# commanderson/morna

Measured on AMD Instinct MI355X. Metric: samples indexed/sec (index build + 1000 queries, k=20) at 50k x 3000, higher is better.
Workload: dtype f32; 1 GPU; synthetic intropolis 50000 samples x 3000 features, 200 trees, 1000 by-item queries, k=20, search_k=100 (BASELINE.json configs[2]); samples_total=50000, samples_per_gpu=50000, features=3000, n_trees=200, queries=1000, k=20, search_k=100, nnz_per_gpu=100542830, junction_lines=70000

## Files before the change

### morna_amd/csrc/knn.hip

```cpp
#include <algorithm>
#include <cfloat>
#include <cstdint>
#include <cmath>
#include <cstring>
#include <type_traits>

#include "common.hpp"
#include "devutil.hpp"
#include "mm16.hpp"

namespace morna {

#define Q_THREADS 256
#define Q_WAVES (Q_THREADS / WAVE)
#define Q_MAX_DPAD 32768
#define Q_LDS_MAX (152 * 1024)

struct QueryParams {
    const float *X;
    const float *norm2;
    int64_t n_items;
    int32_t dpad, n_trees, K;
    const int32_t *node_rec;
    const int32_t *node_tree;
// ... 571 lines not shown
            }
            best = block_min_u64(best, s_red, tid);
            if (tid == 0) emit(r, best);
            prev = best;
        }
    }
    for (int r = kout + tid; r < P.k; r += Q_THREADS) {
        P.ids_out[qi * P.k + r] = -1;
        P.dist_out[qi * P.k + r] = INFINITY;
    }
    if (tid == 0) P.count_out[qi] = kout;
}

template <int BR, int BK, int NS>
__global__ __launch_bounds__(MM16_THREADS) void query_scores_kernel(const _Float16 *__restrict__ X16, int64_t n_items, int32_t dpad,
                                                                    const _Float16 *__restrict__ Q16,
                                                                    const int32_t *__restrict__ qrow, int32_t nq,
                                                                    float *__restrict__ scores, int64_t r_begin )
{
    extern __shared__ __attribute__((aligned(16))) unsigned char smem[];
    __shared__ int32_t s_qrow[MM16_TILE];
    constexpr int NB = BR / 128;
    const int tid = threadIdx.x, lane = tid & (WAVE - 1), w = tid / WAVE;
    const int wm = w >> 1, wn = w & 1;
    const int n_ct = (nq + MM16_TILE - 1) / MM16_TILE;
    const int64_t row_tile = (int64_t)((blockIdx.x >> 3) / n_ct) * 8 + (blockIdx.x & 7);
    const int64_t r0 = r_begin + row_tile * BR;
    const int c0 = (int)((blockIdx.x >> 3) % n_ct) * MM16_TILE;
    if (r0 >= n_items) return;
    if (tid < MM16_TILE) {
        const int q = c0 + tid < nq ? c0 + tid : nq - 1;
        s_qrow[tid] = qrow ? qrow[q] : q;
    }
    __syncthreads();
    mm16_f32x16 acc[NB][2];
    mm16_tile<BR, BK, NS>(X16, Q16, dpad, smem, [&](int rt) { return r0 + rt < n_items ? r0 + rt : n_items - 1; },
                          [&](int rt) { return (int64_t)s_qrow[rt]; }, acc);
    const int lr = lane & 31, lh = lane >> 5;
#pragma unroll
    for (int tb = 0; tb < NB; tb++) {
        const int64_t r = r0 + wm * 32 * NB + tb * 32 + lr;
        if (r < n_items) {
#pragma unroll
            for (int tn = 0; tn < 2; tn++)
#pragma unroll
                for (int e = 0; e < 16; e++) {
                    const int q = c0 + wn * 64 + tn * 32 + (e & 3) + 8 * (e >> 2) + 4 * lh;
                    if (q < nq) scores[(int64_t)q * n_items + r] = acc[tb][tn][e];
                }
        }
    }
}

template <int BK, int NS>
__global__ __launch_bounds__(1024) void query_scores_big_kernel(const _Float16 *__restrict__ X16, int64_t n_items, int32_t dpad,
                                                                const _Float16 *__restrict__ Q16, const int32_t *__restrict__ qrow,
                                                                int32_t nq, float *__restrict__ scores, int32_t n_row_tiles)
{
    extern __shared__ __attribute__((aligned(16))) unsigned char smem[];
    __shared__ int32_t s_qrow[256];
    const int tid = threadIdx.x, lane = tid & (WAVE - 1), w = tid / WAVE;
    const int wm = w >> 2, wn = w & 3;
    const int n_ct = (nq + 255) / 256;
    const int64_t row_tile = (int64_t)((blockIdx.x >> 3) / n_ct) * 8 + (blockIdx.x & 7);
    if (row_tile >= n_row_tiles) return;
    const int64_t r0 = row_tile * 256;
    const int c0 = (int)((blockIdx.x >> 3) % n_ct) * 256;
    if (tid < 256) {
        const int q = c0 + tid < nq ? c0 + tid : nq - 1;
        s_qrow[tid] = qrow ? qrow[q] : q;
    }
    __syncthreads();
    mm16_f32x16 acc[2][2];
    mm16_tile_256x256<BK, NS>(X16, Q16, dpad, smem, [&](int rt) { return r0 + rt; }, [&](int rt) { return (int64_t)s_qrow[rt]; }, acc);
    const int lr = lane & 31, lh = lane >> 5;
#pragma unroll
    for (int tb = 0; tb < 2; tb++) {
        const int64_t r = r0 + wm * 64 + tb * 32 + lr;
#pragma unroll
        for (int tn = 0; tn < 2; tn++)
#pragma unroll
            for (int e = 0; e < 16; e++) {
                const int q = c0 + wn * 64 + tn * 32 + (e & 3) + 8 * (e >> 2) + 4 * lh;
                if (q < nq) scores[(int64_t)q * n_items + r] = acc[tb][tn][e];
            }
    }
}

template <int MODE>
__global__ __launch_bounds__(Q_THREADS) void query_refine_kernel(QueryParams P)
{
    extern __shared__ __attribute__((aligned(16))) unsigned char smem[];
    float4 *qv = (float4 *)smem;
    __shared__ uint64_t s_red[Q_WAVES];
    __shared__ uint64_t s_top[Q_WAVES * KTH_MAX_K];
    __shared__ int s_nsurv;

    const int tid = threadIdx.x, lane = tid & (WAVE - 1), w = tid / WAVE;
    const int64_t qi = blockIdx.x;
    const int nvec = P.dpad / 4;
    const float4 *src = P.items ? (const float4 *)(P.X + (int64_t)P.items[qi] * P.dpad)
                                : (const float4 *)(P.Q + qi * P.dpad);
    for (int i = tid; i < nvec; i += Q_THREADS) qv[i] = src[i];
    if (tid == 0) s_nsurv = 0;
    __syncthreads();

    int32_t *cand = P.cand + qi * P.cap;
    uint64_t *keys = P.keys + qi * P.cap;
    const int ncand = P.ncand[qi] < P.cap ? P.ncand[qi] : P.cap;
    const float pp = P.qpp[qi];
    int nsel = ncand;

    if (MODE != 0 && ncand > P.k) {
        float *low = P.low + qi * P.cap;
        const float nan = __int_as_float(0x7fc00000);
        if (MODE == 1) {
            typedef _Float16 f16x8 __attribute__((ext_vector_type(8)));
            const int nv8 = P.dpad / 8;
            for (int c = w; c < ncand; c += Q_WAVES) {
                const int32_t id = cand[c];
                const f16x8 *y = (const f16x8 *)(P.X16 + (int64_t)id * P.dpad);
                float s0 = 0.f, s1 = 0.f, s2 = 0.f, s3 = 0.f;
                auto mac8 = [&](const f16x8 hv, int i) {
                    const float4 qa = qv[2 * i], qb = qv[2 * i + 1];
                    s0 = fmaf((float)hv[0], qa.x, s0);
                    s1 = fmaf((float)hv[1], qa.y, s1);
                    s2 = fmaf((float)hv[2], qa.z, s2);
                    s3 = fmaf((float)hv[3], qa.w, s3);
                    s0 = fmaf((float)hv[4], qb.x, s0);
                    s1 = fmaf((float)hv[5], qb.y, s1);
                    s2 = fmaf((float)hv[6], qb.z, s2);
                    s3 = fmaf((float)hv[7], qb.w, s3);
                };
                int i = lane;
                for (; i + 5 * WAVE < nv8; i += 6 * WAVE) {
                    const f16x8 h0 = y[i], h1 = y[i + WAVE], h2 = y[i + 2 * WAVE], h3 = y[i + 3 * WAVE];
// ... 292 lines not shown
            uint8_t *dp = (uint8_t *)h->host_small.dev();
            if (!dp) {
                set_error("query: the answer staging is not visible to the device");
                return MORNA_E_HIP;
            }
            P.ids_out = (int32_t *)dp;
            P.dist_out = (float *)(dp + s_ids);
            P.count_out = (int32_t *)(dp + 2 * s_ids);
        }
        if (spread) {
            ScopedTimer tm(h, MORNA_T_QUERY, 0);
            hipLaunchKernelGGL(query_roots_kernel, dim3((unsigned)((h->n_trees + Q_WAVES - 1) / Q_WAVES), (unsigned)nb), dim3(Q_THREADS), 0,
                               h->stream, P);
            MORNA_TRY(launch_descend(h->stream));
#ifdef MORNA_DESCEND_PROBE
            {
                float probe[40];
                HIP_TRY(hipStreamSynchronize(h->stream));
                HIP_TRY(hipMemcpy(probe, P.low + 2 * nb + 16, sizeof(probe), hipMemcpyDeviceToHost));
                fprintf(stderr, "[descend probe] cycles:");
                for (int i = 1; i < (int)probe[0] && i < 40; i++) fprintf(stderr, " %.0f", probe[i]);
                fprintf(stderr, "\n");
            }
#endif
            hipLaunchKernelGGL(query_cand_dots_kernel, dim3((unsigned)((cap + Q_WAVES * QS_CPW - 1) / (Q_WAVES * QS_CPW)), (unsigned)nb),
                               dim3(Q_THREADS), 0, h->stream, P);
            hipLaunchKernelGGL(query_topk_kernel, dim3((unsigned)nb), dim3(Q_THREADS), 0, h->stream, P);
        } else {
            ScopedTimer tm(h, MORNA_T_QUERY, 0);
            if (dense) {
                const _Float16 *q16 = P.X16;
                const int32_t *qrow = P.items;
                if (q_host) {
                    split_mm_convert_rows(h, Qd, nb, Q16, q_n16, q_e16, q_scale, h->stream);
                    q16 = Q16; qrow = nullptr;
                    P.qn16 = q_n16; P.qe16 = q_e16; P.qscale = q_scale;
                } else {
                    P.qn16 = P.xn16; P.qe16 = P.xe16; P.qscale = P.xscale;
                }
                HIP_TRY(hipEventRecord(h->ev_fork, h->stream));
                HIP_TRY(hipStreamWaitEvent(h->stream2, h->ev_fork, 0));
                ScopedTimer tf(h, MORNA_T_QUERY_FILTER, 2 * (int64_t)nb * N * h->dpad);
                static const bool big_on = env_on("MORNA_QUERY_BIG");
                int64_t big_tiles = 0;
                if (big_on && nb >= 512) {
                    const int64_t n_ct_big = (nb + 255) / 256;
                    int64_t a = h->n_cus, b = n_ct_big;
                    while (b) { const int64_t t = a % b; a = b; b = t; }
                    const int64_t per_round = h->n_cus / a;
                    big_tiles = (N / 256) / per_round * per_round;
                }
                if (big_tiles > 0) {
                    const unsigned n_ct_big = (unsigned)((nb + 255) / 256);
                    HIP_TRY(hipFuncSetAttribute((const void *)query_scores_big_kernel<64, 2>, hipFuncAttributeMaxDynamicSharedMemorySize, 128 * 256 * 4));
                    hipLaunchKernelGGL((query_scores_big_kernel<64, 2>), dim3(8u * (unsigned)((big_tiles + 7) / 8) * n_ct_big), dim3(1024), 128 * 256 * 4,
                                       h->stream, P.X16, N, h->dpad, q16, qrow, (int32_t)nb, scores, (int32_t)big_tiles);
                    P.big_rows = big_tiles * 256;
                    P.eacc_big = (4.f * (float)h->dpad + 2.f) * 5.9604645e-8f + 4.1e-6f;
                }
                if (P.big_rows < N) {
                    const unsigned n_ct = (unsigned)((nb + MM16_TILE - 1) / MM16_TILE), n_rt = (unsigned)((N - P.big_rows + 127) / 128);
                    HIP_TRY(hipFuncSetAttribute((const void *)query_scores_kernel<128, 64, 2>, hipFuncAttributeMaxDynamicSharedMemorySize, MM16_LDS));
                    hipLaunchKernelGGL((query_scores_kernel<128, 64, 2>), dim3(8u * ((n_rt + 7) / 8) * n_ct), dim3(MM16_THREADS), MM16_LDS,
                                       big_tiles > 0 ? h->stream2 : h->stream, P.X16, N, h->dpad, q16, qrow, (int32_t)nb, scores, P.big_rows);
                }
                P.scores = scores;
            }
            hipStream_t ts = dense ? h->stream2 : h->stream;
            const int nvq = h->dpad / 256;
            const bool nv_ok = h->dpad % 256 == 0 && (nvq == 1 || nvq == 2 || nvq == 3 || nvq == 4 || nvq == 6 || nvq == 8 || nvq == 12);
            const bool split_traverse = nv_ok && N > h->K && (size_t)QR_Q * h->dpad * 4 <= 128 * 1024 &&
                                        env_on("MORNA_QUERY_SPLIT_TRAVERSE");
            if (split_traverse) {
                const dim3 grid((unsigned)((nb + QR_Q - 1) / QR_Q), (unsigned)((h->n_trees + QR_TREES - 1) / QR_TREES));
                const size_t ql = (size_t)QR_Q * h->dpad * 4;
#define ROOTSB(NVV)                                                                                                      \
    do {                                                                                                                 \
        if (ql > 48 * 1024)                                                                                              \
            HIP_TRY(hipFuncSetAttribute((const void *)query_roots_batch_kernel<NVV>,                                      \
                                        hipFuncAttributeMaxDynamicSharedMemorySize, (int)ql));                           \
        hipLaunchKernelGGL((query_roots_batch_kernel<NVV>), grid, dim3(QR_THREADS), ql, ts, P, (int32_t)nb);             \
    } while (0)
                switch (nvq) {
                case 1: ROOTSB(1); break;
                case 2: ROOTSB(2); break;
                case 3: ROOTSB(3); break;
                case 4: ROOTSB(4); break;
                case 6: ROOTSB(6); break;
                case 8: ROOTSB(8); break;
                default: ROOTSB(12); break;
                }
#undef ROOTSB
                MORNA_TRY(launch_descend(ts));
            } else if (bm_lds) {
                if (lds > 48 * 1024)
                    HIP_TRY(hipFuncSetAttribute((const void *)query_traverse_kernel<true>,
                                                hipFuncAttributeMaxDynamicSharedMemorySize, (int)lds));
                hipLaunchKernelGGL(query_traverse_kernel<true>, dim3((unsigned)nb), dim3(Q_THREADS), lds, ts, P);
            } else {
                if (lds_q > 48 * 1024)
                    HIP_TRY(hipFuncSetAttribute((const void *)query_traverse_kernel<false>,
                                                hipFuncAttributeMaxDynamicSharedMemorySize, (int)lds_q));
                hipLaunchKernelGGL(query_traverse_kernel<false>, dim3((unsigned)nb), dim3(Q_THREADS), lds_q, ts, P);
            }
            if (dense) {
                HIP_TRY(hipEventRecord(h->ev_join, h->stream2));
                HIP_TRY(hipStreamWaitEvent(h->stream, h->ev_join, 0));
            }
#define REFINE(MODE)                                                                                                         \
    do {                                                                                                                     \
        if (lds_q > 48 * 1024)                                                                                               \
// ... 721 lines not shown
```

### morna_amd/csrc/mm16.hpp

```cpp
#pragma once
#include <hip/hip_runtime.h>
#include <stdint.h>

namespace morna {

typedef _Float16 mm16_f16x8 __attribute__((ext_vector_type(8)));
typedef float mm16_f32x16 __attribute__((ext_vector_type(16)));

#define MM16_TILE 128
#define MM16_THREADS 512
#define MM16_LDS_OF(BR, BK, NS) ((NS) * ((BR) + MM16_TILE) * (BK) * 2)
#define MM16_LDS MM16_LDS_OF(128, 64, 2)

#ifndef MM16_PROBE
#define MM16_PROBE 0
#endif
template <int WM, int WN, int NB, int BK, int NS, int CH, typename BRow, typename ARow>
__device__ inline void mm16_core(const _Float16 *__restrict__ B16, const _Float16 *__restrict__ A16, int32_t dpad,
                                 unsigned char *smem, BRow b_row, ARow a_row, mm16_f32x16 (&acc)[NB][2])
{
    static_assert(BK == 32 || BK == 64, "K-step of 32 or 64 halfs");
    constexpr int BR = 32 * NB * WM, AR = 64 * WN, NW = WM * WN;
    constexpr int ROWB = BK * 2;
    constexpr int RPI = 1024 / ROWB;
    constexpr int LPR = ROWB / 16;
    constexpr int STAGE = (BR + AR) * ROWB;
    constexpr int NDMA = (BR + AR) / RPI;
    constexpr int PW = NDMA / NW;
    constexpr int NBLK = BK / 16;
    static_assert(NDMA % NW == 0, "a stage is filled by all waves alike");
    static_assert(PW * (NS - 2) < 64, "vmcnt is a 6-bit counter");
    const int tid = threadIdx.x, lane = tid & 63, w = tid >> 6;
    const int wm = w / WN, wn = w % WN;
    auto swz = [](int row) { return BK == 64 ? (row >> 1) & 7 : (row >> 2) & 3; };
    const _Float16 *src[PW];
#pragma unroll
    for (int u = 0; u < PW; u++) {
        const int j = w * PW + u;
        const bool is_b = j < BR / RPI;
        const int rt = (is_b ? j : j - BR / RPI) * RPI + lane / LPR;
        const int chunk = (lane % LPR) ^ swz(rt);
        src[u] = (is_b ? B16 + (int64_t)b_row(rt) * dpad : A16 + (int64_t)a_row(rt) * dpad) + chunk * 8;
    }
    auto dma = [&](int k0, int stage) {
#pragma unroll
        for (int u = 0; u < PW; u++)
            __builtin_amdgcn_global_load_lds((const __attribute__((address_space(1))) void *)(src[u] + k0),
                                             (__attribute__((address_space(3))) void *)(smem + stage * STAGE + (w * PW + u) * 1024),
                                             16, 0, 0);
    };
    mm16_f32x16 acc_odd[CH == 2 ? NB : 1][2];
#pragma unroll
    for (int i = 0; i < NB; i++)
#pragma unroll
        for (int j = 0; j < 2; j++)
#pragma unroll
            for (int e = 0; e < 16; e++) {
                acc[i][j][e] = 0.f;
                if (CH == 2) acc_odd[i][j][e] = 0.f;
            }

    const int nsteps = dpad / BK;
#pragma unroll
    for (int st = 0; st < NS - 1; st++)
        if (st < nsteps) dma(st * BK, st);
    const int lr = lane & 31, lh = lane >> 5;
    int boff[NB], aoff[2];
#pragma unroll
    for (int tb = 0; tb < NB; tb++) {
        const int brow = wm * 32 * NB + tb * 32 + lr;
        boff[tb] = brow * ROWB + ((lh ^ swz(brow)) << 4);
    }
#pragma unroll
    for (int tn = 0; tn < 2; tn++) {
        const int arow = wn * 64 + tn * 32 + lr;
        aoff[tn] = BR * ROWB + arow * ROWB + ((lh ^ swz(arow)) << 4);
    }
    for (int k = 0; k < nsteps; k++) {
        if (NS > 2 && k + NS - 2 < nsteps) asm volatile("s_waitcnt vmcnt(%0)" ::"n"(PW * (NS - 2)) : "memory");
        else asm volatile("s_waitcnt vmcnt(0)" ::: "memory");
        __syncthreads();
        if (MM16_PROBE != 2 && k + NS - 1 < nsteps) dma((k + NS - 1) * BK, (k + NS - 1) % NS);
        if (MM16_PROBE == 3) continue;
        const unsigned char *st = smem + (k % NS) * STAGE;
        mm16_f16x8 b8[2][NB], a8[2][2];
#pragma unroll
        for (int tb = 0; tb < NB; tb++) b8[0][tb] = *(const mm16_f16x8 *)(st + boff[tb]);
#pragma unroll
        for (int tn = 0; tn < 2; tn++) a8[0][tn] = *(const mm16_f16x8 *)(st + aoff[tn]);
#pragma unroll
        for (int blk = 0; blk < NBLK; blk++) {
            const int cur = blk & 1, nxt = cur ^ 1;
            if (blk + 1 < NBLK) {
#pragma unroll
                for (int tb = 0; tb < NB; tb++) b8[nxt][tb] = *(const mm16_f16x8 *)(st + (boff[tb] ^ ((blk + 1) << 5)));
#pragma unroll
                for (int tn = 0; tn < 2; tn++) a8[nxt][tn] = *(const mm16_f16x8 *)(st + (aoff[tn] ^ ((blk + 1) << 5)));
            }
#pragma unroll
            for (int tb = 0; tb < NB; tb++)
#pragma unroll
                for (int tn = 0; tn < 2; tn++) {
                    if (MM16_PROBE == 1) {
                        acc[tb][tn][0] += (float)a8[cur][tn][0] + (float)b8[cur][tb][0];
                    } else if (CH == 2 && (blk & 1)) acc_odd[tb][tn] = __builtin_amdgcn_mfma_f32_32x32x16_f16(a8[cur][tn], b8[cur][tb], acc_odd[tb][tn], 0, 0, 0);
                    else acc[tb][tn] = __builtin_amdgcn_mfma_f32_32x32x16_f16(a8[cur][tn], b8[cur][tb], acc[tb][tn], 0, 0, 0);
                }
            if (MM16_PROBE == 0 || MM16_PROBE == 2) {
                if (blk + 1 < NBLK) __builtin_amdgcn_sched_group_barrier(0x100, NB + 2, 0);
                __builtin_amdgcn_sched_group_barrier(0x008, 2 * NB, 0);
            }
        }
    }
    __syncthreads();
    if (CH == 2) {
#pragma unroll
        for (int tb = 0; tb < NB; tb++)
#pragma unroll
            for (int tn = 0; tn < 2; tn++) acc[tb][tn] = acc[tb][tn] + acc_odd[tb][tn];
    }
}

template <int BR, int BK, int NS, typename BRow, typename ARow>
__device__ inline void mm16_tile(const _Float16 *__restrict__ B16, const _Float16 *__restrict__ A16, int32_t dpad,
                                 unsigned char *smem, BRow b_row, ARow a_row, mm16_f32x16 (&acc)[BR / 128][2])
{
    mm16_core<4, 2, BR / 128, BK, NS, 2>(B16, A16, dpad, smem, b_row, a_row, acc);
}

template <int BK, int NS, typename BRow, typename ARow>
__device__ inline void mm16_tile_256x256(const _Float16 *__restrict__ B16, const _Float16 *__restrict__ A16, int32_t dpad,
                                         unsigned char *smem, BRow b_row, ARow a_row, mm16_f32x16 (&acc)[2][2])
{
    mm16_core<4, 4, 2, BK, NS, 1>(B16, A16, dpad, smem, b_row, a_row, acc);
}

static inline float mm16_eacc(int32_t dpad) { return (2.f * (float)dpad + 2.f) * 5.9604645e-8f + 4.1e-6f; }

}
```

### morna_amd/csrc/splitmm.hip

```cpp
#include <cstdio>
#include <cstdlib>

#include "common.hpp"
#include "devutil.hpp"
#include "mm16.hpp"

namespace morna {

typedef _Float16 f16x8 __attribute__((ext_vector_type(8)));
typedef float f32x16 __attribute__((ext_vector_type(16)));

static inline float sm_eps(int32_t dpad) { return mm16_eacc(dpad); }

__global__ __launch_bounds__(256) void rows_to_half_kernel(const float *__restrict__ src, int64_t rows, int32_t dpad,
                                                           _Float16 *__restrict__ dst, float *__restrict__ norm,
                                                           float *__restrict__ err ,
                                                           float *__restrict__ inv_scale ,
                                                           unsigned int *__restrict__ zero_me )
{
    if (zero_me && blockIdx.x == 0 && threadIdx.x == 0) *zero_me = 0u;
    const int lane = threadIdx.x & (WAVE - 1);
    const int64_t r = (int64_t)blockIdx.x * (256 / WAVE) + threadIdx.x / WAVE;
    if (r >= rows) return;
    const float4 *x = (const float4 *)(src + r * dpad);
    const int nvec = dpad / 4;
    float m = 0.f;
    bool bad = false;
    for (int i = lane; i < nvec; i += WAVE) {
        const float4 v = x[i];
        const float a = fmaxf(fmaxf(fabsf(v.x), fabsf(v.y)), fmaxf(fabsf(v.z), fabsf(v.w)));
        bad |= !(a <= 3.0e38f);
        m = fmaxf(m, a);
    }
#pragma unroll
    for (int off = 32; off >= 1; off >>= 1) m = fmaxf(m, __shfl_xor(m, off, WAVE));
    bad = __any(bad);
    int e = 0;
    if (m > 0.f) e = 14 - ilogbf(m);
    if (e > 126 || e < -126) bad = true;
    const float s = bad ? 0.f : ldexpf(1.f, e);
    float sum = 0.f, sume = 0.f;
    _Float16 *d = dst + r * dpad;
    for (int i = lane; i < nvec; i += WAVE) {
        const float4 v = x[i];
        const _Float16 h0 = (_Float16)(v.x * s), h1 = (_Float16)(v.y * s), h2 = (_Float16)(v.z * s), h3 = (_Float16)(v.w * s);
        typedef _Float16 f16x4 __attribute__((ext_vector_type(4)));
        *(f16x4 *)(d + 4 * i) = (f16x4){h0, h1, h2, h3};
        const float f0 = (float)h0, f1 = (float)h1, f2 = (float)h2, f3 = (float)h3;
        sum += (f0 * f0 + f1 * f1) + (f2 * f2 + f3 * f3);
        const float e0 = v.x * s - f0, e1 = v.y * s - f1, e2 = v.z * s - f2, e3 = v.w * s - f3;
        sume += (e0 * e0 + e1 * e1) + (e2 * e2 + e3 * e3);
    }
    sum = wave_sum_xor(sum);
    sume = wave_sum_xor(sume);
    if (lane == 0) {
        norm[r] = bad ? INFINITY : sqrtf(sum) * 1.002f;
        err[r] = bad ? 0.f : sqrtf(sume) * 1.002f + 1e-30f;
        if (inv_scale) inv_scale[r] = bad ? 0.f : ldexpf(1.f, -e);
    }
}

#define SM_OPEN 1408

template <bool BIG>
__global__ __launch_bounds__(BIG ? 1024 : 512) void split_mm_kernel(
    const _Float16 *__restrict__ X16, const float *__restrict__ xn, const float *__restrict__ xe, int64_t n_items, int32_t dpad,
    const _Float16 *__restrict__ H16, const float *__restrict__ hn, const float *__restrict__ he, int32_t n_tasks,
    const SplitTask *__restrict__ tasks, const int32_t *__restrict__ inv ,
    const int32_t *__restrict__ item_at ,
    float eps, uint8_t *__restrict__ side, int32_t *__restrict__ ones, unsigned int *__restrict__ amb_count,
    int2 *__restrict__ amb, unsigned int amb_cap,
    const int32_t *__restrict__ col_list ,
    const int32_t *__restrict__ col_count ,
    const int32_t *__restrict__ col_first )
{
    constexpr int ROWS = BIG ? 256 : 128, COLS = ROWS, THREADS = BIG ? 1024 : 512;
    extern __shared__ __attribute__((aligned(16))) unsigned char smem[];
    float *Cs = (float *)smem;
    __shared__ int s_ones[COLS], s_tree[COLS], s_start[COLS], s_end[COLS], s_task[COLS], s_slot[COLS];
    __shared__ float s_hn[COLS], s_he[COLS];
    __shared__ int2 s_open[SM_OPEN];
    __shared__ int s_nopen;
    __shared__ unsigned int s_obase;
    const int tid = threadIdx.x, lane = tid & (WAVE - 1), w = tid / WAVE;
    const int n_ct = (n_tasks + COLS - 1) / COLS;
    int64_t row_tile;
    int c0;
    if (col_list) {
        const int n_rt = (int)((n_items + ROWS - 1) / ROWS);
        const int total = col_first[n_rt], run = (total + 7) / 8;
        const int slot = (int)(blockIdx.x >> 3), g = (int)(blockIdx.x & 7) * run + slot;
        if (slot >= run || g >= total) return;
        int lo = 0, hi = n_rt - 1;
        while (lo < hi) {
            const int mid = (lo + hi + 1) >> 1;
            if (col_first[mid] <= g) lo = mid;
            else hi = mid - 1;
        }
        row_tile = lo;
        c0 = (g - col_first[lo]) * COLS;
    } else {
        row_tile = (int64_t)((blockIdx.x >> 3) / n_ct) * 8 + (blockIdx.x & 7);
        c0 = (int)((blockIdx.x >> 3) % n_ct) * COLS;
    }
    const int64_t r0 = row_tile * ROWS;
    if (r0 >= n_items) return;
    const int n_mine = col_list ? col_count[row_tile] : n_tasks;
    if (c0 >= n_mine) return;
    const int n_valid = n_mine - c0 < COLS ? n_mine - c0 : COLS;
    if (tid < COLS) {
        const int k = c0 + (tid < n_valid ? tid : n_valid - 1);
        const int col = col_list ? col_list[row_tile * n_tasks + k] : k;
        const SplitTask t = tasks[col];
        s_ones[tid] = 0;
        if (tid == 0) s_nopen = 0;
        s_task[tid] = col;
        s_slot[tid] = t.slot;
        s_tree[tid] = t.tree;
        s_start[tid] = t.start;
        s_end[tid] = t.start + t.count;
        s_hn[tid] = hn[t.slot];
        s_he[tid] = he[t.slot];
    }
    __syncthreads();
    constexpr int NB = BIG ? 2 : 1;
    f32x16 acc[NB][2];
    auto b_row = [&](int rt) {
        const int64_t r = r0 + rt < n_items ? r0 + rt : n_items - 1;
        return item_at ? (int64_t)item_at[r] : r;
    };
    auto a_row = [&](int rt) { return (int64_t)s_slot[rt]; };
    if constexpr (BIG) mm16_tile_256x256<64, 2>(X16, H16, dpad, smem, b_row, a_row, acc);
    else mm16_tile<128, 64, 2>(X16, H16, dpad, smem, b_row, a_row, acc);
    const int lr = lane & 31, lh = lane >> 5;
    const int wm = BIG ? w >> 2 : w >> 1, wn = BIG ? w & 3 : w & 1;

    const int64_t row = r0 + (tid & (ROWS - 1));
    const bool row_ok = row < n_items;
    const int64_t item = row_ok ? (item_at ? (int64_t)item_at[row] : row) : 0;
    const float xn_r = xn[item], xe_r = xe[item];
    const float xa = (eps * xn_r + xe_r) * 1.005f, xb = (xn_r + xe_r) * 1.005f;
#pragma unroll
    for (int half = 0; half < COLS / 128; half++) {
        if (half) __syncthreads();
        if ((wn >> 1) == half) {
#pragma unroll
            for (int tb = 0; tb < NB; tb++)
#pragma unroll
                for (int tn = 0; tn < 2; tn++)
#pragma unroll
                    for (int e = 0; e < 16; e++)
                        Cs[((wn & 1) * 64 + tn * 32 + (e & 3) + 8 * (e >> 2) + 4 * lh) * ROWS + wm * 32 * NB + tb * 32 + lr] = acc[tb][tn][e];
        }
        __syncthreads();
        const int c_lo = half * 128;
        if (c_lo >= n_valid) break;
        const int c_hi = (c_lo + 128 < n_valid ? c_lo + 128 : n_valid);
        const int t_first = s_tree[c_lo], t_last = s_tree[c_hi - 1];
        constexpr int EU = BIG ? 4 : 8, TSTEP = THREADS / ROWS;
        for (int tb = t_first + tid / ROWS; tb <= t_last; tb += EU * TSTEP) {
            int a[EU], pos[EU], pp[EU];
#pragma unroll
            for (int u = 0; u < EU; u++) {
                const int tr = tb + u * TSTEP;
                pp[u] = (row_ok && tr <= t_last) ? inv[(int64_t)tr * n_items + row] : -1;
            }
#pragma unroll
            for (int u = 0; u < EU; u++) {
                const int tr = tb + u * TSTEP;
                a[u] = -1;
                pos[u] = 0;
                int lo = -1, n_t = 0;
#pragma unroll
                for (int k = 0; k < COLS / WAVE; k++) {
                    const uint64_t mk = __ballot(k * WAVE + lane < n_valid && s_tree[k * WAVE + lane] == tr);
                    if (mk && lo < 0) lo = k * WAVE + (int)__builtin_ctzll(mk);
                    n_t += (int)__builtin_popcountll(mk);
                }
                int before = 0;
                for (int j = 0; j < n_t; j++) before += s_start[lo + j] <= pp[u] ? 1 : 0;
                if (pp[u] >= 0 && before > 0 && pp[u] < s_end[lo + before - 1]) {
                    a[u] = lo + before - 1;
                    pos[u] = pp[u] - s_start[lo + before - 1];
                }
            }
#pragma unroll
            for (int u = 0; u < EU; u++) {
                const int tr = tb + u * TSTEP;
                const bool mine = a[u] >= c_lo && a[u] < c_hi;
                const int cl = mine ? a[u] : 0;
                const float c = Cs[(mine ? a[u] - c_lo : 0) * ROWS + (tid & (ROWS - 1))];
                const bool decided = mine && fabsf(c) > xa * s_hn[cl] + xb * s_he[cl];
                const bool one = decided && c > 0.f;
                if (decided) side[(int64_t)tr * n_items + s_start[cl] + pos[u]] = (uint8_t)one;
                const uint64_t mm = __ballot(mine);
                if (mm) {
                    const int cl0 = __builtin_amdgcn_readlane(cl, __builtin_ctzll(mm));
                    const uint64_t onem = __ballot(one);
                    if (__ballot(mine && cl != cl0) == 0) {
                        if (onem && lane == __builtin_ctzll(mm)) atomicAdd(&s_ones[cl0], (int)__builtin_popcountll(onem));
                    } else if (one) {
                        atomicAdd(&s_ones[cl], 1);
                    }
                }
                const bool open = mine && !decided;
                const uint64_t om = __ballot(open);
                if (om) {
                    int base = 0;
                    if (lane == __builtin_ctzll(om)) base = atomicAdd(&s_nopen, (int)__builtin_popcountll(om));
                    base = __builtin_amdgcn_readlane(base, __builtin_ctzll(om));
                    const int idx = base + (int)__builtin_popcountll(om & ((1ull << lane) - 1ull));
                    if (open) {
// ... 237 lines not shown
    *rank_out = rank;
    *inv_out = invr.p;
    return MORNA_OK;
}

int split_mm_prepare_rows(morna_index *h, hipStream_t stream)
{
    if (h->half.valid) return MORNA_OK;
    DevBuf<_Float16> &x16 = h->half.x16;
    DevBuf<float> &xn = h->half.xn;
    MORNA_TRY(x16.alloc((size_t)h->n_items * h->dpad));
    MORNA_TRY(xn.alloc((size_t)h->n_items * 3));
    hipLaunchKernelGGL(rows_to_half_kernel, dim3((unsigned)((h->n_items + 3) / 4)), dim3(256), 0, stream, h->X.p,
                       h->n_items, h->dpad, x16.p, xn.p, xn.p + 2 * h->n_items, xn.p + h->n_items, (unsigned int *)nullptr);
    HIP_TRY(hipGetLastError());
    h->half.valid = true;
    return MORNA_OK;
}

int split_mm_convert_rows(morna_index *h, const float *src, int64_t rows, _Float16 *dst, float *norm, float *err,
                          float *inv_scale, hipStream_t stream)
{
    hipLaunchKernelGGL(rows_to_half_kernel, dim3((unsigned)((rows + 3) / 4)), dim3(256), 0, stream, src, rows, h->dpad, dst,
                       norm, err, inv_scale, (unsigned int *)nullptr);
    HIP_TRY(hipGetLastError());
    return MORNA_OK;
}

int split_mm_level(morna_index *h, const SplitTask *d_tasks, int32_t n_tasks, int32_t n_slots, const float *hp_level,
                   const int32_t *perm, const int32_t *inv, uint32_t seed, uint8_t *side, int32_t *ones)
{
    const int64_t N = h->n_items;
    DevBuf<_Float16> &h16 = h->splitmm.h16;
    DevBuf<float> &hn = h->splitmm.hn;
    DevBuf<uint8_t> &ambuf = h->splitmm.amb;
    const bool ord = h->splitmm.ord_valid;
    const _Float16 *rows16 = h->half.x16.p;
    const float *rows_n = h->half.xn.p, *rows_e = h->half.xn.p + 2 * N;
    const int32_t *rank = ord ? h->splitmm.maps.p : nullptr, *item_at = ord ? h->splitmm.maps.p + N : nullptr;
    const size_t cap = (size_t)N * h->n_trees;
    if (cap > 0xFFFFFFF0u) {
        set_error("split_mm_level: %lld x %d (row, tree) pairs exceed the open-pair list", (long long)N, h->n_trees);
        return MORNA_E_INVALID;
    }
    MORNA_TRY(h16.alloc((size_t)n_slots * h->dpad));
    MORNA_TRY(hn.alloc((size_t)n_slots * 2));
    MORNA_TRY(ambuf.alloc(16 + cap * sizeof(int2)));
    unsigned int *amb_count = (unsigned int *)ambuf.p;
    int2 *amb = (int2 *)(ambuf.p + 16);
    hipLaunchKernelGGL(rows_to_half_kernel, dim3((unsigned)((n_slots + 3) / 4)), dim3(256), 0, h->stream, hp_level,
                       (int64_t)n_slots, h->dpad, h16.p, hn.p, hn.p + n_slots, (float *)nullptr, amb_count);
    static const bool big_on = env_on("MORNA_SPLIT_BIG");
    static const bool lists_on = env_on("MORNA_SPLIT_LISTS");
    if (big_on && (n_tasks >= 1024 || (ord && lists_on && n_tasks >= 512))) {
        const unsigned n_rt = (unsigned)((N + 255) / 256), n_ct = (unsigned)((n_tasks + 255) / 256);
        const int32_t *col_list = nullptr, *col_count = nullptr, *col_first = nullptr;
        if (lists_on) {
            DevBuf<uint8_t> &active = h->splitmm.active;
            DevBuf<int32_t> &lists = h->splitmm.lists;
            MORNA_TRY(active.alloc((size_t)n_rt * n_tasks));
            MORNA_TRY(lists.alloc((size_t)n_rt * n_tasks + 2 * n_rt + 1));
            HIP_TRY(hipMemsetAsync(active.p, 0, (size_t)n_rt * n_tasks, h->stream));
            hipLaunchKernelGGL(split_active_mark_kernel, dim3((unsigned)n_tasks), dim3(256), 0, h->stream, d_tasks, perm, N, rank, 8,
                               n_tasks, active.p);
            hipLaunchKernelGGL(split_active_list_kernel, dim3(n_rt), dim3(256), 0, h->stream, active.p, n_tasks, lists.p,
                               lists.p + (size_t)n_rt * n_tasks);
            col_list = lists.p;
            col_count = lists.p + (size_t)n_rt * n_tasks;
            const bool count_tiles = h->timing && (h->timing_mask & (1u << MORNA_T_SPLIT_MM));
            hipLaunchKernelGGL(split_active_scan_kernel, dim3(1), dim3(1024), 0, h->stream, col_count, (int32_t)n_rt, 256,
                               lists.p + (size_t)n_rt * n_tasks + n_rt, count_tiles ? h->d_stat.p + 1 : (unsigned long long *)nullptr);
            col_first = col_count + n_rt;
        }
        ScopedTimer tmm(h, MORNA_T_SPLIT_MM, lists_on ? 0 : 2ll * 256 * 256 * h->dpad * (int64_t)n_rt * n_ct);
        const float eps1 = (4.f * (float)h->dpad + 2.f) * 5.9604645e-8f + 4.1e-6f;
        HIP_TRY(hipFuncSetAttribute((const void *)split_mm_kernel<true>, hipFuncAttributeMaxDynamicSharedMemorySize, 128 * 256 * 4));
        hipLaunchKernelGGL(split_mm_kernel<true>, dim3(8u * ((n_rt + 7) / 8) * n_ct), dim3(1024), 128 * 256 * 4, h->stream, rows16, rows_n,
                           rows_e, N, h->dpad, h16.p, hn.p, hn.p + n_slots, n_tasks, d_tasks, inv, item_at, eps1, side, ones,
                           amb_count, amb, (unsigned int)cap, col_list, col_count, col_first);
    } else {
        const unsigned n_rt = (unsigned)((N + 127) / 128), n_ct = (unsigned)((n_tasks + 127) / 128);
        static_assert(MM16_LDS == 128 * 128 * 4, "the slabs and the result tile share the dynamic LDS");
        HIP_TRY(hipFuncSetAttribute((const void *)split_mm_kernel<false>, hipFuncAttributeMaxDynamicSharedMemorySize, 128 * 128 * 4));
        ScopedTimer tmm(h, MORNA_T_SPLIT_MM, 2ll * 128 * 128 * h->dpad * (int64_t)n_rt * n_ct);
        hipLaunchKernelGGL(split_mm_kernel<false>, dim3(8u * ((n_rt + 7) / 8) * n_ct), dim3(512), 128 * 128 * 4, h->stream, rows16, rows_n,
                           rows_e, N, h->dpad, h16.p, hn.p, hn.p + n_slots, n_tasks, d_tasks, inv, item_at, sm_eps(h->dpad), side,
                           ones, amb_count, amb, (unsigned int)cap, (const int32_t *)nullptr, (const int32_t *)nullptr, (const int32_t *)nullptr);
    }
    hipLaunchKernelGGL(split_amb_kernel, dim3((unsigned)(4 * h->n_cus)), dim3(256), 0, h->stream, h->X.p, N, h->dpad, d_tasks,
                       inv, seed, hp_level, amb_count, amb, (unsigned int)cap, side, ones, item_at);
    HIP_TRY(hipGetLastError());
    static const bool debug_open = getenv("MORNA_DEBUG_OPEN") && atoi(getenv("MORNA_DEBUG_OPEN")) != 0;
    if (debug_open) {
        unsigned int n_open = 0;
        HIP_TRY(hipStreamSynchronize(h->stream));
        HIP_TRY(hipMemcpy(&n_open, amb_count, 4, hipMemcpyDeviceToHost));
        fprintf(stderr, "[morna] split_mm level: D=%d split nodes=%d (row, tree) pairs<=%lld open=%u (%.4f %%)\n", h->dim,
                n_tasks, (long long)cap, n_open, 100.0 * n_open / (double)cap);
    }
    return MORNA_OK;
}

}
```

Before: 7.357 million samples/s.

## Replace 1024-thread 256x256 fp16 GEMM tile with 512-thread multi-phase LDS pipeline

Adds mm16_pipe256, a 256x256 fp16 MFMA tile computed by 8 waves. It keeps an 8-slot LDS ring filled through direct global-to-LDS loads, with a configurable number of loads in flight. Each wave now holds a 4x2 accumulator block, and compute is split into per-half phases separated by barriers, with raised wave priority around the MFMAs. The query big-score kernel and the big split GEMM kernel switch to it. Their shared tables move into dynamic LDS, and the output index mapping is updated to match. The goal is to overlap memory latency with matrix work and halve the thread count, at the cost of more registers per wave and complex barrier choreography. Both paths stay behind environment switches, and a new MORNA_SPLIT_BIG_MIN threshold is added.

```diff
diff --git a/morna_amd/csrc/knn.hip b/morna_amd/csrc/knn.hip
--- a/morna_amd/csrc/knn.hip
+++ b/morna_amd/csrc/knn.hip
@@ -647,13 +647,13 @@
     }
 }
 
-template <int BK, int NS>
-__global__ __launch_bounds__(1024) void query_scores_big_kernel(const _Float16 *__restrict__ X16, int64_t n_items, int32_t dpad,
-                                                                const _Float16 *__restrict__ Q16, const int32_t *__restrict__ qrow,
-                                                                int32_t nq, float *__restrict__ scores, int32_t n_row_tiles)
+#define QSB_LDS (MM16_PIPE_LDS + 256 * 4)
+__global__ __launch_bounds__(MM16_PIPE_THREADS) void query_scores_big_kernel(const _Float16 *__restrict__ X16, int64_t n_items, int32_t dpad,
+                                                                             const _Float16 *__restrict__ Q16, const int32_t *__restrict__ qrow,
+                                                                             int32_t nq, float *__restrict__ scores, int32_t n_row_tiles)
 {
     extern __shared__ __attribute__((aligned(16))) unsigned char smem[];
-    __shared__ int32_t s_qrow[256];
+    int32_t *s_qrow = (int32_t *)(smem + MM16_PIPE_LDS);
     const int tid = threadIdx.x, lane = tid & (WAVE - 1), w = tid / WAVE;
     const int wm = w >> 2, wn = w & 3;
     const int n_ct = (nq + 255) / 256;
@@ -666,17 +666,17 @@
         s_qrow[tid] = qrow ? qrow[q] : q;
     }
     __syncthreads();
-    mm16_f32x16 acc[2][2];
-    mm16_tile_256x256<BK, NS>(X16, Q16, dpad, smem, [&](int rt) { return r0 + rt; }, [&](int rt) { return (int64_t)s_qrow[rt]; }, acc);
+    mm16_f32x16 acc[4][2];
+    mm16_pipe256(X16, Q16, dpad, smem, [&](int rt) { return r0 + rt; }, [&](int rt) { return (int64_t)s_qrow[rt]; }, acc);
     const int lr = lane & 31, lh = lane >> 5;
 #pragma unroll
-    for (int tb = 0; tb < 2; tb++) {
-        const int64_t r = r0 + wm * 64 + tb * 32 + lr;
+    for (int tb = 0; tb < 4; tb++) {
+        const int64_t r = r0 + (tb >> 1) * 128 + wm * 64 + (tb & 1) * 32 + lr;
 #pragma unroll
         for (int tn = 0; tn < 2; tn++)
 #pragma unroll
             for (int e = 0; e < 16; e++) {
-                const int q = c0 + wn * 64 + tn * 32 + (e & 3) + 8 * (e >> 2) + 4 * lh;
+                const int q = c0 + tn * 128 + wn * 32 + (e & 3) + 8 * (e >> 2) + 4 * lh;
                 if (q < nq) scores[(int64_t)q * n_items + r] = acc[tb][tn][e];
             }
     }
@@ -1075,11 +1075,11 @@
                 }
                 if (big_tiles > 0) {
                     const unsigned n_ct_big = (unsigned)((nb + 255) / 256);
-                    HIP_TRY(hipFuncSetAttribute((const void *)query_scores_big_kernel<64, 2>, hipFuncAttributeMaxDynamicSharedMemorySize, 128 * 256 * 4));
-                    hipLaunchKernelGGL((query_scores_big_kernel<64, 2>), dim3(8u * (unsigned)((big_tiles + 7) / 8) * n_ct_big), dim3(1024), 128 * 256 * 4,
+                    HIP_TRY(hipFuncSetAttribute((const void *)query_scores_big_kernel, hipFuncAttributeMaxDynamicSharedMemorySize, QSB_LDS));
+                    hipLaunchKernelGGL(query_scores_big_kernel, dim3(8u * (unsigned)((big_tiles + 7) / 8) * n_ct_big), dim3(MM16_PIPE_THREADS), QSB_LDS,
                                        h->stream, P.X16, N, h->dpad, q16, qrow, (int32_t)nb, scores, (int32_t)big_tiles);
                     P.big_rows = big_tiles * 256;
-                    P.eacc_big = (4.f * (float)h->dpad + 2.f) * 5.9604645e-8f + 4.1e-6f;
+                    P.eacc_big = mm16_eacc_one(h->dpad);
                 }
                 if (P.big_rows < N) {
                     const unsigned n_ct = (unsigned)((nb + MM16_TILE - 1) / MM16_TILE), n_rt = (unsigned)((N - P.big_rows + 127) / 128);
diff --git a/morna_amd/csrc/mm16.hpp b/morna_amd/csrc/mm16.hpp
--- a/morna_amd/csrc/mm16.hpp
+++ b/morna_amd/csrc/mm16.hpp
@@ -29,7 +29,7 @@
     constexpr int PW = NDMA / NW;
     constexpr int NBLK = BK / 16;
     static_assert(NDMA % NW == 0, "a stage is filled by all waves alike");
-    static_assert(PW * (NS - 2) < 64, "vmcnt is a 6-bit counter");
+    static_assert(NS == 2, "behind __syncthreads() no delivery survives the barrier: more stages only cost LDS (see mm16_pipe256)");
     const int tid = threadIdx.x, lane = tid & 63, w = tid >> 6;
     const int wm = w / WN, wn = w % WN;
     auto swz = [](int row) { return BK == 64 ? (row >> 1) & 7 : (row >> 2) & 3; };
@@ -77,8 +77,7 @@
         aoff[tn] = BR * ROWB + arow * ROWB + ((lh ^ swz(arow)) << 4);
     }
     for (int k = 0; k < nsteps; k++) {
-        if (NS > 2 && k + NS - 2 < nsteps) asm volatile("s_waitcnt vmcnt(%0)" ::"n"(PW * (NS - 2)) : "memory");
-        else asm volatile("s_waitcnt vmcnt(0)" ::: "memory");
+        asm volatile("s_waitcnt vmcnt(0)" ::: "memory");
         __syncthreads();
         if (MM16_PROBE != 2 && k + NS - 1 < nsteps) dma((k + NS - 1) * BK, (k + NS - 1) % NS);
         if (MM16_PROBE == 3) continue;
@@ -128,13 +127,135 @@
     mm16_core<4, 2, BR / 128, BK, NS, 2>(B16, A16, dpad, smem, b_row, a_row, acc);
 }
 
-template <int BK, int NS, typename BRow, typename ARow>
-__device__ inline void mm16_tile_256x256(const _Float16 *__restrict__ B16, const _Float16 *__restrict__ A16, int32_t dpad,
-                                         unsigned char *smem, BRow b_row, ARow a_row, mm16_f32x16 (&acc)[2][2])
+#define MM16_PIPE_THREADS 512
+#define MM16_PIPE_LDS (8 * 16384)
+#ifndef MM16_PIPE_FLY
+#define MM16_PIPE_FLY 3
+#endif
+template <int V> struct mm16_int { static constexpr int value = V; };
+
+template <typename BRow, typename ARow>
+__device__ inline void mm16_pipe256(const _Float16 *__restrict__ B16, const _Float16 *__restrict__ A16, int32_t dpad,
+                                    unsigned char *smem, BRow b_row, ARow a_row, mm16_f32x16 (&acc)[4][2])
 {
-    mm16_core<4, 4, 2, BK, NS, 1>(B16, A16, dpad, smem, b_row, a_row, acc);
+    constexpr int FLY = MM16_PIPE_FLY, LOOK = FLY + 1, HALF = 16384;
+    static_assert(FLY >= 1 && FLY <= 5, "a slot is refilled two phases behind its read at the earliest");
+    const int tid = threadIdx.x, lane = tid & 63;
+    const int w = __builtin_amdgcn_readfirstlane(tid >> 6);
+    const int wm = w >> 2, wn = w & 3;
+    const int lr = lane & 31, lh = lane >> 5;
+    auto swz = [](int row) { return (row >> 1) & 7; };
+    const _Float16 *src[4][2];
+#pragma unroll
+    for (int i = 0; i < 4; i++)
+#pragma unroll
+        for (int u = 0; u < 2; u++) {
+            const int rh = (w * 2 + u) * 8 + (lane >> 3);
+            const int rt = ((i == 1 || i == 2) ? 128 : 0) + rh;
+            const int chunk = (lane & 7) ^ swz(rh);
+            src[i][u] = ((i & 1) == 0 ? B16 + (int64_t)b_row(rt) * dpad : A16 + (int64_t)a_row(rt) * dpad) + chunk * 8;
+        }
+    auto issue = [&](auto S8, int kstep) {
+        constexpr int slot = decltype(S8)::value, i = slot & 3;
+#pragma unroll
+        for (int u = 0; u < 2; u++)
+            __builtin_amdgcn_global_load_lds((const __attribute__((address_space(1))) void *)(src[i][u] + (int64_t)kstep * 64),
+                                             (__attribute__((address_space(3))) void *)(smem + slot * HALF + (w * 2 + u) * 1024),
+                                             16, 0, 0);
+    };
+#pragma unroll
+    for (int tb = 0; tb < 4; tb++)
+#pragma unroll
+        for (int tn = 0; tn < 2; tn++)
+#pragma unroll
+            for (int e = 0; e < 16; e++) acc[tb][tn][e] = 0.f;
+    int boff[2], aoff;
+#pragma unroll
+    for (int t2 = 0; t2 < 2; t2++) {
+        const int row = wm * 64 + t2 * 32 + lr;
+        boff[t2] = row * 128 + ((lh ^ swz(row)) << 4);
+    }
+    {
+        const int row = wn * 32 + lr;
+        aoff = row * 128 + ((lh ^ swz(row)) << 4);
+    }
+    mm16_f16x8 b8[2][4], a8[2][4];
+
+    auto phase = [&](auto PH, auto ISSUE, auto NFLY, int t) {
+        constexpr int P = decltype(PH)::value, j = P & 3, par = P >> 2;
+        const unsigned char *st = smem + P * HALF;
+        if constexpr (j == 0 || j == 2) {
+#pragma unroll
+            for (int t2 = 0; t2 < 2; t2++) {
+                int o = boff[t2];
+                asm volatile("" : "+v"(o));
+#pragma unroll
+                for (int blk = 0; blk < 4; blk++) b8[t2][blk] = *(const mm16_f16x8 *)(st + (o ^ (blk << 5)));
+            }
+        } else if (decltype(NFLY)::value >= 0) {
+            int o = aoff;
+            asm volatile("" : "+v"(o));
+#pragma unroll
+            for (int blk = 0; blk < 4; blk++) a8[par ^ 1][blk] = *(const mm16_f16x8 *)(st + (o ^ (blk << 5)));
+        }
+        if constexpr (decltype(ISSUE)::value) {
+            constexpr int S8 = (P + LOOK) & 7;
+            issue(mm16_int<S8>{}, t + ((j + LOOK) >> 2) + ((S8 & 3) == 3 ? 1 : 0));
+        }
+        if constexpr (decltype(NFLY)::value >= 0) asm volatile("s_waitcnt vmcnt(%0)" ::"n"(2 * decltype(NFLY)::value) : "memory");
+        __builtin_amdgcn_s_barrier();
+        asm volatile("s_waitcnt lgkmcnt(0)" ::: "memory");
+        __builtin_amdgcn_sched_barrier(0);
+        __builtin_amdgcn_s_setprio(1);
+        constexpr int tb0 = j < 2 ? 0 : 2, tn = (j == 1 || j == 2) ? 1 : 0, as = tn ? par ^ 1 : par;
+#pragma unroll
+        for (int blk = 0; blk < 4; blk++)
+#pragma unroll
+            for (int t2 = 0; t2 < 2; t2++)
+                acc[tb0 + t2][tn] = __builtin_amdgcn_mfma_f32_32x32x16_f16(a8[as][blk], b8[t2][blk], acc[tb0 + t2][tn], 0, 0, 0);
+        __builtin_amdgcn_s_setprio(0);
+        __builtin_amdgcn_sched_barrier(0);
+        __builtin_amdgcn_s_barrier();
+    };
+
+    const int nsteps = dpad / 64;
+    issue(mm16_int<7>{}, 0);
+    issue(mm16_int<0>{}, 0);
+    if constexpr (LOOK > 1) issue(mm16_int<1>{}, 0);
+    if constexpr (LOOK > 2) issue(mm16_int<2>{}, 0);
+    if constexpr (LOOK > 3) issue(mm16_int<3>{}, 1);
+    if constexpr (LOOK > 4) issue(mm16_int<4>{}, 1);
+    if constexpr (LOOK > 5) issue(mm16_int<5>{}, 1);
+    asm volatile("s_waitcnt vmcnt(%0)" ::"n"(2 * FLY) : "memory");
+    __builtin_amdgcn_s_barrier();
+#pragma unroll
+    for (int blk = 0; blk < 4; blk++) a8[0][blk] = *(const mm16_f16x8 *)(smem + 7 * HALF + (aoff ^ (blk << 5)));
+    asm volatile("s_waitcnt lgkmcnt(0)" ::: "memory");
+    __builtin_amdgcn_sched_barrier(0);
+    if (wm == 1) __builtin_amdgcn_s_barrier();
+
+    typedef mm16_int<1> yes;
+    typedef mm16_int<FLY> fly;
+    int t = 0;
+    for (; t < nsteps - 2; t += 2) {
+        phase(mm16_int<0>{}, yes{}, fly{}, t);
+        phase(mm16_int<1>{}, yes{}, fly{}, t);
+        phase(mm16_int<2>{}, yes{}, fly{}, t);
+        phase(mm16_int<3>{}, yes{}, fly{}, t);
+        phase(mm16_int<4>{}, yes{}, fly{}, t + 1);
+        phase(mm16_int<5>{}, yes{}, fly{}, t + 1);
+        phase(mm16_int<6>{}, yes{}, fly{}, t + 1);
+        phase(mm16_int<7>{}, yes{}, fly{}, t + 1);
+    }
+#define MM16_TAIL(i) phase(mm16_int<i>{}, mm16_int<(i + LOOK <= 6)>{}, \
+                           mm16_int<(i == 7 ? -1 : ((i + LOOK < 6 ? i + LOOK : 6) - (i + 1) > 0 ? (i + LOOK < 6 ? i + LOOK : 6) - (i + 1) : 0))>{}, t + (i >> 2))
+    MM16_TAIL(0); MM16_TAIL(1); MM16_TAIL(2); MM16_TAIL(3); MM16_TAIL(4); MM16_TAIL(5); MM16_TAIL(6); MM16_TAIL(7);
+#undef MM16_TAIL
+    if (wm == 0) __builtin_amdgcn_s_barrier();
+    __syncthreads();
 }
 
 static inline float mm16_eacc(int32_t dpad) { return (2.f * (float)dpad + 2.f) * 5.9604645e-8f + 4.1e-6f; }
-
-}
+static inline float mm16_eacc_one(int32_t dpad) { return (4.f * (float)dpad + 2.f) * 5.9604645e-8f + 4.1e-6f; }
+
+}
diff --git a/morna_amd/csrc/splitmm.hip b/morna_amd/csrc/splitmm.hip
--- a/morna_amd/csrc/splitmm.hip
+++ b/morna_amd/csrc/splitmm.hip
@@ -62,8 +62,10 @@
 
 #define SM_OPEN 1408
 
+#define SM_TABLES (8 * 256 * 4 + SM_OPEN * 8 + 16)
+#define SM_BIG_LDS (MM16_PIPE_LDS + SM_TABLES)
 template <bool BIG>
-__global__ __launch_bounds__(BIG ? 1024 : 512) void split_mm_kernel(
+__global__ __launch_bounds__(512) void split_mm_kernel(
     const _Float16 *__restrict__ X16, const float *__restrict__ xn, const float *__restrict__ xe, int64_t n_items, int32_t dpad,
     const _Float16 *__restrict__ H16, const float *__restrict__ hn, const float *__restrict__ he, int32_t n_tasks,
     const SplitTask *__restrict__ tasks, const int32_t *__restrict__ inv ,
@@ -74,14 +76,32 @@
     const int32_t *__restrict__ col_count ,
     const int32_t *__restrict__ col_first )
 {
-    constexpr int ROWS = BIG ? 256 : 128, COLS = ROWS, THREADS = BIG ? 1024 : 512;
+    constexpr int ROWS = BIG ? 256 : 128, COLS = ROWS, THREADS = 512;
     extern __shared__ __attribute__((aligned(16))) unsigned char smem[];
     float *Cs = (float *)smem;
-    __shared__ int s_ones[COLS], s_tree[COLS], s_start[COLS], s_end[COLS], s_task[COLS], s_slot[COLS];
-    __shared__ float s_hn[COLS], s_he[COLS];
-    __shared__ int2 s_open[SM_OPEN];
-    __shared__ int s_nopen;
-    __shared__ unsigned int s_obase;
+    int *s_ones, *s_tree, *s_start, *s_end, *s_task, *s_slot;
+    float *s_hn, *s_he;
+    int2 *s_open;
+    int *p_nopen;
+    unsigned int *p_obase;
+    if constexpr (BIG) {
+        int *tb = (int *)(smem + MM16_PIPE_LDS);
+        s_ones = tb; s_tree = tb + COLS; s_start = tb + 2 * COLS; s_end = tb + 3 * COLS; s_task = tb + 4 * COLS; s_slot = tb + 5 * COLS;
+        s_hn = (float *)(tb + 6 * COLS); s_he = (float *)(tb + 7 * COLS);
+        s_open = (int2 *)(tb + 8 * COLS);
+        p_nopen = (int *)(s_open + SM_OPEN);
+        p_obase = (unsigned int *)(p_nopen + 1);
+    } else {
+        __shared__ int t_ones[COLS], t_tree[COLS], t_start[COLS], t_end[COLS], t_task[COLS], t_slot[COLS];
+        __shared__ float t_hn[COLS], t_he[COLS];
+        __shared__ int2 t_open[SM_OPEN];
+        __shared__ int t_nopen;
+        __shared__ unsigned int t_obase;
+        s_ones = t_ones; s_tree = t_tree; s_start = t_start; s_end = t_end; s_task = t_task; s_slot = t_slot;
+        s_hn = t_hn; s_he = t_he; s_open = t_open; p_nopen = &t_nopen; p_obase = &t_obase;
+    }
+    int &s_nopen = *p_nopen;
+    unsigned int &s_obase = *p_obase;
     const int tid = threadIdx.x, lane = tid & (WAVE - 1), w = tid / WAVE;
     const int n_ct = (n_tasks + COLS - 1) / COLS;
     int64_t row_tile;
@@ -123,41 +143,47 @@
         s_he[tid] = he[t.slot];
     }
     __syncthreads();
-    constexpr int NB = BIG ? 2 : 1;
+    constexpr int NB = BIG ? 4 : 1;
     f32x16 acc[NB][2];
     auto b_row = [&](int rt) {
         const int64_t r = r0 + rt < n_items ? r0 + rt : n_items - 1;
         return item_at ? (int64_t)item_at[r] : r;
     };
     auto a_row = [&](int rt) { return (int64_t)s_slot[rt]; };
-    if constexpr (BIG) mm16_tile_256x256<64, 2>(X16, H16, dpad, smem, b_row, a_row, acc);
+    const int64_t row = r0 + (tid & (ROWS - 1));
+    const bool row_ok = row < n_items;
+    if constexpr (BIG) mm16_pipe256(X16, H16, dpad, smem, b_row, a_row, acc);
     else mm16_tile<128, 64, 2>(X16, H16, dpad, smem, b_row, a_row, acc);
     const int lr = lane & 31, lh = lane >> 5;
     const int wm = BIG ? w >> 2 : w >> 1, wn = BIG ? w & 3 : w & 1;
 
-    const int64_t row = r0 + (tid & (ROWS - 1));
-    const bool row_ok = row < n_items;
     const int64_t item = row_ok ? (item_at ? (int64_t)item_at[row] : row) : 0;
     const float xn_r = xn[item], xe_r = xe[item];
     const float xa = (eps * xn_r + xe_r) * 1.005f, xb = (xn_r + xe_r) * 1.005f;
 #pragma unroll
     for (int half = 0; half < COLS / 128; half++) {
         if (half) __syncthreads();
-        if ((wn >> 1) == half) {
+        if constexpr (BIG) {
 #pragma unroll
             for (int tb = 0; tb < NB; tb++)
 #pragma unroll
-                for (int tn = 0; tn < 2; tn++)
-#pragma unroll
-                    for (int e = 0; e < 16; e++)
-                        Cs[((wn & 1) * 64 + tn * 32 + (e & 3) + 8 * (e >> 2) + 4 * lh) * ROWS + wm * 32 * NB + tb * 32 + lr] = acc[tb][tn][e];
+                for (int e = 0; e < 16; e++) {
+                    const f32x16 &v = half ? acc[tb][1] : acc[tb][0];
+                    Cs[(wn * 32 + (e & 3) + 8 * (e >> 2) + 4 * lh) * ROWS + (tb >> 1) * 128 + wm * 64 + (tb & 1) * 32 + lr] = v[e];
+                }
+        } else {
+#pragma unroll
+            for (int tn = 0; tn < 2; tn++)
+#pragma unroll
+                for (int e = 0; e < 16; e++)
+                    Cs[(wn * 64 + tn * 32 + (e & 3) + 8 * (e >> 2) + 4 * lh) * ROWS + wm * 32 + lr] = acc[0][tn][e];
         }
         __syncthreads();
         const int c_lo = half * 128;
         if (c_lo >= n_valid) break;
         const int c_hi = (c_lo + 128 < n_valid ? c_lo + 128 : n_valid);
         const int t_first = s_tree[c_lo], t_last = s_tree[c_hi - 1];
-        constexpr int EU = BIG ? 4 : 8, TSTEP = THREADS / ROWS;
+        constexpr int EU = 8, TSTEP = THREADS / ROWS;
         for (int tb = t_first + tid / ROWS; tb <= t_last; tb += EU * TSTEP) {
             int a[EU], pos[EU], pp[EU];
 #pragma unroll
@@ -501,7 +527,8 @@
                        (int64_t)n_slots, h->dpad, h16.p, hn.p, hn.p + n_slots, (float *)nullptr, amb_count);
     static const bool big_on = env_on("MORNA_SPLIT_BIG");
     static const bool lists_on = env_on("MORNA_SPLIT_LISTS");
-    if (big_on && (n_tasks >= 1024 || (ord && lists_on && n_tasks >= 512))) {
+    static const int big_min = getenv("MORNA_SPLIT_BIG_MIN") ? atoi(getenv("MORNA_SPLIT_BIG_MIN")) : -1;
+    if (big_on && (big_min >= 0 ? n_tasks >= big_min : (n_tasks >= 1024 || (ord && lists_on && n_tasks >= 512)))) {
         const unsigned n_rt = (unsigned)((N + 255) / 256), n_ct = (unsigned)((n_tasks + 255) / 256);
         const int32_t *col_list = nullptr, *col_count = nullptr, *col_first = nullptr;
         if (lists_on) {
@@ -522,9 +549,10 @@
             col_first = col_count + n_rt;
         }
         ScopedTimer tmm(h, MORNA_T_SPLIT_MM, lists_on ? 0 : 2ll * 256 * 256 * h->dpad * (int64_t)n_rt * n_ct);
-        const float eps1 = (4.f * (float)h->dpad + 2.f) * 5.9604645e-8f + 4.1e-6f;
-        HIP_TRY(hipFuncSetAttribute((const void *)split_mm_kernel<true>, hipFuncAttributeMaxDynamicSharedMemorySize, 128 * 256 * 4));
-        hipLaunchKernelGGL(split_mm_kernel<true>, dim3(8u * ((n_rt + 7) / 8) * n_ct), dim3(1024), 128 * 256 * 4, h->stream, rows16, rows_n,
+        const float eps1 = mm16_eacc_one(h->dpad);
+        static_assert(MM16_PIPE_LDS == 128 * 256 * 4, "the staging ring and the result tile share the dynamic LDS");
+        HIP_TRY(hipFuncSetAttribute((const void *)split_mm_kernel<true>, hipFuncAttributeMaxDynamicSharedMemorySize, SM_BIG_LDS));
+        hipLaunchKernelGGL(split_mm_kernel<true>, dim3(8u * ((n_rt + 7) / 8) * n_ct), dim3(MM16_PIPE_THREADS), SM_BIG_LDS, h->stream, rows16, rows_n,
                            rows_e, N, h->dpad, h16.p, hn.p, hn.p + n_slots, n_tasks, d_tasks, inv, item_at, eps1, side, ones,
                            amb_count, amb, (unsigned int)cap, col_list, col_count, col_first);
     } else {
```

Result: slower. 7.261 million samples/s (-1.3%).
